# fabian-sp/GGLasso

Measured on AMD Instinct MI355X. Metric: ADMM iters/sec on (K=32,p=500) GGL at 1/2/4/8 GPUs; eigh HBM GB/s vs peak, higher is better.
Workload: dtype f64

## Files before the change

### gglasso_amd/csrc/capi_ops.hip

```cpp
#include "capi_internal.hpp"

static int eig_common(int K, int p, const double* A, const double* beta, double* D, double* Q, double* out, int map,
                      int eig_method)
{
    ARGCHK(K >= 1 && p >= 1 && A, "K, p, A");
    ARGCHK(eig_method != GGL_EIG_JACOBI || jacobi_fits(p), "GGL_EIG_JACOBI needs p <= GGL_JACOBI_MAX_P");
    const bool jac = (eig_method == GGL_EIG_JACOBI) || (eig_method == GGL_EIG_AUTO && jacobi_fits(p));
    const size_t n = (size_t)K * p * p, kp = (size_t)K * p;
    DevBuf dA, dD, dR, dO, dB, dE, dS;
    int* dinfo = nullptr;
    HIPCHK(dA.alloc(n));
    HIPCHK(dD.alloc(kp));
    HIPCHK(dB.alloc(K));
    HIPCHK(hipMalloc(&dinfo, K * sizeof(int)));
    struct InfoFree { int* p; ~InfoFree() { (void)hipFree(p); } } infofree{dinfo};
    UP(dA.p, A, n);
    if (beta) UP(dB.p, beta, K);
    if (out) HIPCHK(dO.alloc(n));
    std::vector<int> info(K);
    if (jac) {
        if (Q) HIPCHK(dR.alloc(n));
        HIPCHK(launch_jacobi(nullptr, dA.p, dD.p, dR.p, dO.p, map, beta ? dB.p : nullptr, dinfo, K, p));
        HIPCHK(hipDeviceSynchronize());
        HIPCHK(hipMemcpy(info.data(), dinfo, K * sizeof(int), hipMemcpyDeviceToHost));
// ... 120 lines not shown
    std::vector<double> h(n), coef((size_t)K * NS_NCOEF, 0.0);
    unsigned long long s = 88172645463325252ull;
    for (size_t i = 0; i < n; ++i) {
        s ^= s << 13; s ^= s >> 7; s ^= s << 17;
        h[i] = (double)(s >> 11) / 9007199254740992.0 - 0.5;
    }
    for (int k = 0; k < K; ++k) coef[(size_t)k * NS_NCOEF + 1] = 1.0 / p;
    DevBuf dA, dB, dC, dcoef;
    HIPCHK(dA.alloc(n));
    HIPCHK(dB.alloc(n));
    HIPCHK(dC.alloc(n));
    HIPCHK(dcoef.alloc(coef.size()));
    UP(dA.p, h.data(), n);
    UP(dB.p, h.data(), n);
    UP(dcoef.p, coef.data(), coef.size());
    hipEvent_t e0, e1;
    HIPCHK(hipEventCreate(&e0));
    HIPCHK(hipEventCreate(&e1));
    for (int i = 0; i < 3; ++i) launch_symm(nullptr, dA.p, dB.p, dC.p, nullptr, nullptr, dcoef.p, K, p, variant);
    HIPCHK(hipEventRecord(e0, nullptr));
    for (int i = 0; i < iters; ++i) launch_symm(nullptr, dA.p, dB.p, dC.p, nullptr, nullptr, dcoef.p, K, p, variant);
    HIPCHK(hipEventRecord(e1, nullptr));
    HIPCHK(hipEventSynchronize(e1));
    float ms = 0.f;
    HIPCHK(hipEventElapsedTime(&ms, e0, e1));
    (void)hipEventDestroy(e0);
    (void)hipEventDestroy(e1);
    HIPCHK(hipGetLastError());
    *ms_out = ms / iters;
    return GGL_OK;
}

#ifdef GGL_DEV
extern "C" int ggl_dev_set_symm_epilogue(int serial) { return symm_set_serial_epilogue(serial != 0) ? 1 : 0; }

extern "C" int ggl_dev_symm_bench_ops(int K, int p, int variant, int iters, int ops, double* ms_out)
{
    ARGCHK(K >= 1 && p >= 1 && iters >= 1 && ms_out && ops >= 0 && ops <= 7, "arguments");
    ARGCHK(variant < 0 || symm_variant_built(variant), "product-kernel variant not in this build");
    const size_t n = (size_t)K * p * p;
    std::vector<double> h(n), coef((size_t)K * NS_NCOEF, 0.0);
    unsigned long long s = 88172645463325252ull;
    for (size_t i = 0; i < n; ++i) {
        s ^= s << 13; s ^= s >> 7; s ^= s << 17;
        h[i] = (double)(s >> 11) / 9007199254740992.0 - 0.5;
    }
    for (int k = 0; k < K; ++k)
        for (int i = 0; i < p; ++i)
            for (int j = 0; j < i; ++j) h[((size_t)k * p + i) * p + j] = h[((size_t)k * p + j) * p + i];
    for (int k = 0; k < K; ++k) {
        double* c = coef.data() + (size_t)k * NS_NCOEF;
        c[0] = 1.5; c[1] = 1.0 / p; c[2] = -0.5; c[3] = 0.25; c[4] = 0.5; c[5] = 0.125; c[6] = 0.75; c[7] = -0.375;
    }
    DevBuf dA, dB, dC, dC2, dcoef;
    HIPCHK(dA.alloc(n));
    HIPCHK(dB.alloc(n));
    HIPCHK(dC.alloc(n));
    HIPCHK(dC2.alloc(n));
    HIPCHK(dcoef.alloc(coef.size()));
    UP(dA.p, h.data(), n);
    UP(dB.p, h.data(), n);
    UP(dcoef.p, coef.data(), coef.size());
    const double* E = (ops & 1) ? dA.p : nullptr;
    const double* E2 = (ops & 2) ? dB.p : nullptr;
    double* C2 = (ops & 4) ? dC2.p : nullptr;
    struct Events {
        hipEvent_t e0 = nullptr, e1 = nullptr;
// ... 907 lines not shown
```

### gglasso_amd/csrc/gemm_sym.hip

```cpp
#include <algorithm>
#include <initializer_list>
#include <mutex>
#include <unordered_map>
#include <type_traits>

#include "common.hpp"
#include "kernels.hpp"
#include "sym_tile.hpp"

namespace ggl {


__device__ __forceinline__ double c2val(double dC, double v, double dE, double e) { return __builtin_fma(dE, e, dC * v); }
__device__ __forceinline__ double c2val2(double dC, double v, double dE, double e, bool has2, double dE2, double f)
{
    const double w = c2val(dC, v, dE, e);
    return has2 ? __builtin_fma(dE2, f, w) : w;
}


template <int BM, int BK, int WM, int WN, bool LM, int ABL = 0>
__global__ __launch_bounds__(sym_nt(BM, WM, WN)) void k_symm_tn(
    const double* __restrict__ A, const double* __restrict__ B, double* __restrict__ C, double* __restrict__ C2,
    const double* __restrict__ E, const double* __restrict__ coef, int K, int p, const double* __restrict__ A1,
    const double* __restrict__ B1, double* __restrict__ C1, int K1, double* __restrict__ maxdev,
    const double* __restrict__ E2)
{
    using Cfg = SymCfg<BM, BK, WM, WN, LM>;
    __shared__ __attribute__((aligned(16))) double smem[Cfg::LDS_DOUBLES];
    double* As = smem;
    double* Bs = smem + Cfg::SLAB;
    const int T = (p + BM - 1) / BM;
    int k, b;
    if (!decode_block_xcd(T * (T + 1) / 2, K + K1, k, b)) return;
    const bool second = k >= K;
    const int kk = second ? k - K : k;
    int I = 0;
    while (b >= T - I) { b -= T - I; ++I; }
    const int J = I + b;
    const int I0 = I * BM, J0 = J * BM;
    const int tid = threadIdx.x, lane = tid & 63, wave = tid >> 6;
    const int wr = (wave / Cfg::NWC) * WM, wc = (wave % Cfg::NWC) * WN;
    const size_t pp = (size_t)p * p;
    const double* Ak = (second ? A1 : A) + (size_t)kk * pp;
    const double* Bk = (second ? B1 : B) + (size_t)kk * pp;

#ifdef GGL_DEV
    long long t_start = 0, t_loop = 0, t_loop_end = 0;
    if (ABL == 3) t_start = clock64();
#endif

    v4d acc[Cfg::TI][Cfg::TJ];
// ... 304 lines not shown
            for (int j = 0; j < IPW; ++j) {
                const int i = wave * IPW + j;
                const unsigned ro = min((unsigned)(m0 + RPI * i + lrow), pm1) * pu;
                double* la = base + j * 128;
                __builtin_amdgcn_global_load_lds((gptr_t)(Ak + ro + ca), (lptr_t)la, 16, 0, AUX);
                __builtin_amdgcn_global_load_lds((gptr_t)(Bk + ro + cb), (lptr_t)(la + SLAB), 16, 0, AUX);
            }
        }
    };
    constexpr bool REBAL = (TI == 2 && TJ == 2 && NW == 4);
    int rbk[TI], cbk[TJ];
#pragma unroll
    for (int i = 0; i < TI; ++i) rbk[i] = wr + 16 * i;
#pragma unroll
    for (int j = 0; j < TJ; ++j) cbk[j] = wc + 16 * j;
    const bool skipU = REBAL && I == J;
    int nval = TI * TJ;
    if (skipU) {
        nval = 3;
        if (wave == 1) { cbk[0] = wc + 16; cbk[TJ - 1] = wc; }
        else if (wave == 2) { rbk[0] = 16; rbk[TI - 1] = 0; cbk[0] = WN + 16; cbk[TJ - 1] = WN; nval = 1; }
    }
    const bool dead_wave = !REBAL && (I == J) && (wr >= wc + WN);
    double cI = 0.0, cAcc = 0.0, cE = 0.0, dI = 0.0, dC = 0.0, dE = 0.0, cE2 = 0.0, dE2 = 0.0;
    double* Ck = (second ? C1 : C) + (size_t)kk * pp;
    double* C2k = (C2 && !second) ? C2 + (size_t)kk * pp : nullptr;
    const double* Ek = (E && !second) ? E + (size_t)kk * pp : nullptr;
    const double* E2k = (E2 && !second) ? E2 + (size_t)kk * pp : nullptr;
    auto load_coefs = [&] {
        cI = coef[k * NS_NCOEF + 0]; cAcc = coef[k * NS_NCOEF + 1]; cE = coef[k * NS_NCOEF + 2];
        dI = coef[k * NS_NCOEF + 3]; dC = coef[k * NS_NCOEF + 4]; dE = coef[k * NS_NCOEF + 5];
        cE2 = E2k ? coef[k * NS_NCOEF + 6] : 0.0; dE2 = E2k ? coef[k * NS_NCOEF + 7] : 0.0;
    };
    if constexpr (SER == 0 && ABL != 4) load_coefs();
    const int S = (p + BK - 1) / BK;
#pragma unroll
    for (int q = 0; q < NSTG - 1; ++q)
        if (q < S) issue(q, q);
    const int fg = lane >> 4, fsw = 16 * (fg & 1);
    const double* pfa[TI];
    const double* pfb[TJ];
#pragma unroll
    for (int i = 0; i < TI; ++i) pfa[i] = smem + fg * BM + ((rbk[i] + (lane & 15)) ^ fsw);
#pragma unroll
    for (int j = 0; j < TJ; ++j) pfb[j] = smem + SLAB + fg * BM + ((cbk[j] + (lane & 15)) ^ fsw);
    auto slab = [&](const int s, auto bufc) {
        constexpr int buf = decltype(bufc)::value;
        const int ahead = min(NSTG - 2, S - 1 - s);
        if (NSTG >= 6 && ahead >= 4) wait_vmcnt<(NSTG >= 6 ? 8 * IPW : 0)>();
        else if (NSTG >= 5 && ahead >= 3) wait_vmcnt<(NSTG >= 5 ? 6 * IPW : 0)>();
        else if (NSTG >= 4 && ahead >= 2) wait_vmcnt<4 * IPW>();
        else if (NSTG >= 3 && ahead >= 1) wait_vmcnt<2 * IPW>();
        else wait_vmcnt<0>();
        const int valid = p - s * BK;
        if (valid < BK) {
            for (int e = lane; e < RPW * BM; e += 64) {
                const int row = wave * RPW + e / BM;
                if (row >= valid) {
                    smem[(size_t)buf * 2 * SLAB + row * BM + (e % BM)] = 0.0;
                    smem[(size_t)buf * 2 * SLAB + SLAB + row * BM + (e % BM)] = 0.0;
                }
            }
        }
        asm volatile("s_waitcnt lgkmcnt(0)" ::: "memory");
        if (ABL != 5) __builtin_amdgcn_s_barrier();
        asm volatile("" ::: "memory");
        if (s + NSTG - 1 < S) issue(s + NSTG - 1, (buf + NSTG - 1) % NSTG);
// ... 11 lines not shown
                for (int i = 0; i < TI; ++i) af[i] = pfa[i][so + kq4 * 4 * BM];
#pragma unroll
                for (int j = 0; j < TJ; ++j) bf[j] = pfb[j][so + kq4 * 4 * BM];
                if constexpr (REBAL && ABL != 3) {
                    if (!skipU) acc[TI - 1][0] = __builtin_amdgcn_mfma_f64_16x16x4f64(af[TI - 1], bf[0], acc[TI - 1][0], 0, 0, 0);
                    acc[0][0] = __builtin_amdgcn_mfma_f64_16x16x4f64(af[0], bf[0], acc[0][0], 0, 0, 0);
                    acc[0][TJ - 1] = __builtin_amdgcn_mfma_f64_16x16x4f64(af[0], bf[TJ - 1], acc[0][TJ - 1], 0, 0, 0);
                    acc[TI - 1][TJ - 1] = __builtin_amdgcn_mfma_f64_16x16x4f64(af[TI - 1], bf[TJ - 1], acc[TI - 1][TJ - 1], 0, 0, 0);
                } else {
#pragma unroll
                    for (int i = 0; i < TI; ++i)
#pragma unroll
                        for (int j = 0; j < TJ; ++j) {
                            if (ABL == 3) { acc[i][j][0] += af[i] * bf[j]; continue; }
                            acc[i][j] = __builtin_amdgcn_mfma_f64_16x16x4f64(af[i], bf[j], acc[i][j], 0, 0, 0);
                        }
                }
            }
#if defined(GGL_EXP_SETPRIO) && GGL_EXP_SETPRIO == 1
            __builtin_amdgcn_s_setprio(0);
#endif
        }
    };
    auto stages = [&](const int s0, auto... bufs) {
        (void)std::initializer_list<int>{((s0 + (int)decltype(bufs)::value < S) ? (slab(s0 + (int)decltype(bufs)::value, bufs), 0) : 0)...};
    };
    static_assert(NSTG == 2 || NSTG == 3 || NSTG == 4 || NSTG == 6, "stage counts with an unrolled slab loop");
    for (int s0 = 0; s0 < S; s0 += NSTG) {
        if constexpr (NSTG == 2) stages(s0, std::integral_constant<int, 0>{}, std::integral_constant<int, 1>{});
        else if constexpr (NSTG == 3) stages(s0, std::integral_constant<int, 0>{}, std::integral_constant<int, 1>{}, std::integral_constant<int, 2>{});
        else if constexpr (NSTG == 4) stages(s0, std::integral_constant<int, 0>{}, std::integral_constant<int, 1>{}, std::integral_constant<int, 2>{}, std::integral_constant<int, 3>{});
        else stages(s0, std::integral_constant<int, 0>{}, std::integral_constant<int, 1>{}, std::integral_constant<int, 2>{}, std::integral_constant<int, 3>{}, std::integral_constant<int, 4>{}, std::integral_constant<int, 5>{});
    }
    if constexpr (ABL == 4 || SER != 0) __syncthreads();
#if defined(GGL_EXP_SETPRIO) && GGL_EXP_SETPRIO == 2
    __builtin_amdgcn_s_setprio(2);
#endif
    if (ABL == 4) {
        double keepalive = 0.0;
#pragma unroll
        for (int i = 0; i < TI; ++i)
#pragma unroll
            for (int j = 0; j < TJ; ++j) keepalive += acc[i][j][0] + acc[i][j][1] + acc[i][j][2] + acc[i][j][3];
        if (keepalive == 1234.5678) C[0] = keepalive;
        return;
    }

#ifdef GGL_DEV
    if constexpr (SER != 0) {
        load_coefs();
        double dev = 0.0;
        const bool wide = (I != J) && ABL != 1;
        if (wide) {
    #pragma unroll
            for (int ti = 0; ti < TI; ++ti)
    #pragma unroll
                for (int tj = 0; tj < TJ; ++tj)
    #pragma unroll
                    for (int r = 0; r < 4; ++r) {
                        const int row = wr + ti * 16 + (lane >> 4) + 4 * r;
                        const int col = wc + tj * 16 + (lane & 15);
                        smem[row * BM + (col ^ row)] = cAcc * acc[ti][tj][r];
                    }
            __syncthreads();
            auto ld2 = [](const double* q) { return *reinterpret_cast<const double2*>(q); };
            auto lde2 = [&](const double* q) {
                if constexpr (AUX == 0) return *reinterpret_cast<const double2*>(q);
                else { double2 e; e.x = ld_pol<AUX>(q); e.y = ld_pol<AUX>(q + 1); return e; }
            };
            for (int e2 = tid; e2 < BM * BM / 2; e2 += NT) {
                const int row = e2 / (BM / 2), c2 = (e2 % (BM / 2)) * 2;
                const int gi = I0 + row, gj = J0 + c2;
                double2 t = ld2(smem + row * BM + ((c2 ^ row) & ~1));
                if (row & 1) { const double h = t.x; t.x = t.y; t.y = h; }
                if (gi < p && gj + 1 < p) {
                    double2 e = {0.0, 0.0}, f = {0.0, 0.0};
                    if (Ek) e = lde2(Ek + (size_t)gi * p + gj);
                    if (E2k) f = lde2(E2k + (size_t)gi * p + gj);
                    double2 v;
                    v.x = t.x + cE * e.x;
                    v.y = t.y + cE * e.y;
                    if (E2k) { v.x += cE2 * f.x; v.y += cE2 * f.y; }
// ... 108 lines not shown
                    const double f0 = need_f ? ld_pol<AUX>(E2k + (size_t)(J0 + a) * p + I0 + c2) : 0.0;
                    if (!rowpart) { v0 += cE * e0; if (E2k) v0 += cE2 * f0; }
                    Ck[(size_t)(J0 + a) * p + I0 + c2] = v0;
                    if (C2k) C2k[(size_t)(J0 + a) * p + I0 + c2] = c2val2(dC, v0, dE, e0, E2k != nullptr, dE2, f0);
                }
            }
        }
        return;
    }
#endif
    constexpr int LDSB = NSTG * 2 * SLAB * 8;
    constexpr int WGCU = (160 * 1024 / LDSB) < (8 / (NW / 4)) ? (160 * 1024 / LDSB) : (8 / (NW / 4));
    constexpr int VBUD = (512 / (WGCU * (NW / 4))) & ~7;
    constexpr int BREG = VBUD - TI * TJ * 8 - 48 - XREG;
    constexpr int NTRIP = BM * BM / 2 / NT;
    constexpr int NB = (BREG / 8 >= NTRIP) ? NTRIP : (BREG / 8 >= NTRIP / 2 && NTRIP >= 2) ? NTRIP / 2 : 1;
    constexpr int NBLK = TI * TJ;
    constexpr int DB = (BREG / 16 >= NBLK) ? NBLK : (BREG / 16 >= NBLK / 2 && NBLK >= 2) ? NBLK / 2 : 1;
    static_assert(NTRIP * NT * 2 == BM * BM && NTRIP % NB == 0 && NBLK % DB == 0, "epilogue batches");
    auto lds_barrier = [] {
        asm volatile("s_waitcnt lgkmcnt(0)" ::: "memory");
        __builtin_amdgcn_s_barrier();
        asm volatile("" ::: "memory");
    };
    auto landed = [](const double& x) { asm volatile("" ::"v"(x)); };
    auto landed2 = [&](const double2& x) { landed(x.x); landed(x.y); };
    auto ld2 = [](const double* q) { return *reinterpret_cast<const double2*>(q); };
    auto lde2 = [&](const double* q) {
        if constexpr (AUX == 0) return *reinterpret_cast<const double2*>(q);
        else { double2 e; e.x = ld_pol<AUX>(q); e.y = ld_pol<AUX>(q + 1); return e; }
    };
    double dev = 0.0;
    const bool wide = (I != J) && ABL != 1;
    if (wide) {
        double2 pe[NB], pf[NB];
        auto direct_loads = [&](const int u0) {
#pragma unroll
            for (int q = 0; q < NB; ++q) {
                const int e2 = tid + (u0 + q) * NT;
                const int row = e2 / (BM / 2), c2 = (e2 % (BM / 2)) * 2;
                const int gi = I0 + row, gj = J0 + c2;
                const bool any = gi < p && gj < p, half = any && gj + 1 >= p;
                const size_t o = (size_t)gi * p + gj - (half ? 1 : 0);
                pe[q] = double2{0.0, 0.0};
                pf[q] = double2{0.0, 0.0};
                if (any) {
                    if (Ek) pe[q] = lde2(Ek + o);
                    if (E2k) pf[q] = lde2(E2k + o);
                }
            }
        };
        direct_loads(0);
        lds_barrier();
#pragma unroll
        for (int ti = 0; ti < TI; ++ti)
#pragma unroll
            for (int tj = 0; tj < TJ; ++tj)
#pragma unroll
                for (int r = 0; r < 4; ++r) {
                    const int row = wr + ti * 16 + (lane >> 4) + 4 * r;
                    const int col = wc + tj * 16 + (lane & 15);
                    smem[row * BM + (col ^ row)] = cAcc * acc[ti][tj][r];
                }
        lds_barrier();
#pragma unroll
        for (int u0 = 0; u0 < NTRIP; u0 += NB) {
            if (u0 > 0) direct_loads(u0);
// ... 82 lines not shown
            for (int q = 0; q < DB; ++q) {
                const int ti = (b0 + q) / TJ, tj = (b0 + q) % TJ;
                if (no_block(ti, tj)) continue;
#pragma unroll
                for (int r = 0; r < 4; ++r) {
                    const int row = rbk[ti] + (lane >> 4) + 4 * r;
                    const int col = cbk[tj] + (lane & 15);
                    const int gi = I0 + row, gj = J0 + col;
                    double v = cAcc * acc[ti][tj][r];
                    const bool keep = gi < p && gj < p && (I != J || gi <= gj);
                    if (keep) {
                        if (gi == gj) v += cI;
                        const double e0 = de[q * 4 + r], f0 = df[q * 4 + r];
                        v = __builtin_fma(cE, e0, v);
                        if (E2k) v = __builtin_fma(cE2, f0, v);
                        dev = fmax(dev, fabs(v - (gi == gj ? 1.0 : 0.0)));
                        Ck[(size_t)gi * p + gj] = v;
                        if (C2k) C2k[(size_t)gi * p + gj] = c2val2(dC, v, dE, e0, E2k != nullptr, dE2, f0) + (gi == gj ? dI : 0.0);
                        if (I == J && gi != gj) {
                            Ck[(size_t)gj * p + gi] = v;
                            if (C2k) C2k[(size_t)gj * p + gi] = c2val2(dC, v, dE, e0, E2k != nullptr, dE2, f0);
                        }
                    }
                    if ((I != J || rowpart) && ABL != 1) smem[row * BM + (col ^ row)] = (rowpart && !keep) ? 0.0 : v;
                }
            }
        }
    }
    if (maxdev) {
        dev = wave_max(dev);
        if (lane == 0 && dev > 0.0)
            atomicMax(reinterpret_cast<unsigned long long*>(maxdev + k), (unsigned long long)__double_as_longlong(dev));
    }
    if ((I != J || rowpart) && ABL != 1) lds_barrier();
    if (rowpart && ABL != 1 && tid < 2 * BM) symm_dl_partials<BM>(smem, rowpart, fropart, k, p, T, blockTile, I, J, I0, J0, tid);
    if (wide) {
        const bool need_e = Ek && C2k && (!rowpart || dE != 0.0), need_f = E2k && C2k && (!rowpart || dE2 != 0.0);
        double2 me[NB], mf[NB];
#pragma unroll
        for (int u0 = 0; u0 < NTRIP; u0 += NB) {
#pragma unroll
            for (int q = 0; q < NB; ++q) {
                const int e2 = tid + (u0 + q) * NT;
                const int a = e2 / (BM / 2), c2 = (e2 % (BM / 2)) * 2;
                const size_t o = (size_t)(J0 + a) * p + I0 + c2;
                const bool any = J0 + a < p && I0 + c2 < p, half = any && I0 + c2 + 1 >= p;
                me[q] = double2{0.0, 0.0};
                mf[q] = double2{0.0, 0.0};
                if (any) {
                    if (need_e) me[q] = lde2(Ek + o - (half ? 1 : 0));
                    if (need_f) mf[q] = lde2(E2k + o - (half ? 1 : 0));
                }
            }
#pragma unroll
            for (int q = 0; q < NB; ++q) { landed2(me[q]); landed2(mf[q]); }
#pragma unroll
            for (int q = 0; q < NB; ++q) {
                const int e2 = tid + (u0 + q) * NT;
                const int a = e2 / (BM / 2), c2 = (e2 % (BM / 2)) * 2;
                const size_t o = (size_t)(J0 + a) * p + I0 + c2;
                double2 e = me[q], f = mf[q];
                if (J0 + a < p && I0 + c2 < p && I0 + c2 + 1 >= p) { e.x = e.y; f.x = f.y; }
                if (J0 + a < p && I0 + c2 + 1 < p) {
                    double2 v;
                    v.x = smem[c2 * BM + (a ^ c2)];
                    v.y = smem[(c2 + 1) * BM + (a ^ (c2 + 1))];
                    *reinterpret_cast<double2*>(Ck + o) = v;
                    if (C2k) {
                        double2 w;
// ... 461 lines not shown
                    if (Ek && dE != 0.0) e = *reinterpret_cast<const double2*>(Ek + (size_t)gm * p + gc);
                    double2 w2;
                    w2.x = c2val(dC, v.x, dE, e.x);
                    w2.y = c2val(dC, v.y, dE, e.y);
                    *reinterpret_cast<double2*>(C2k + (size_t)gm * p + gc) = w2;
                }
            }
        }
    }
    if (rowpart && tid < 2 * BM) {
        const int t = tid & (BM - 1);
        const bool second = tid >= BM;
        double rs = 0.0, sq = 0.0;
        if (!second) {
#pragma unroll 8
            for (int c = 0; c < BM; ++c) { const double x = smem[t * BM + ((c + t) & (BM - 1))]; rs += fabs(x); sq += x * x; }
        } else if (I != J) {
#pragma unroll 8
            for (int r = 0; r < BM; ++r) rs += fabs(smem[((r + t) & (BM - 1)) * BM + t]);
        }
        if (I != J) sq *= 2.0;
        if (I != J || !second) {
            const int slot = second ? I : J, gr = (second ? J0 : I0) + t;
            if (gr < p) rowpart[((size_t)k * T + slot) * (size_t)p + gr] = rs;
        }
        sq = wave_sum(second ? 0.0 : sq);
        if (tid == 0) fropart[(size_t)k * (T * (T + 1) / 2) + blockTile] = sq;
    }
}

#endif

#ifdef GGL_DEV
static bool g_symm_serial = false;
bool symm_set_serial_epilogue(bool on) { const bool was = g_symm_serial; g_symm_serial = on; return was; }
#endif

#ifdef GGL_DEV
template <int BK, int NSTG, int BM, int AUX, int SER = 0>
__global__ __launch_bounds__(256) void k_omega_chain(const ChainProg P, unsigned* __restrict__ state)
{
    __shared__ __attribute__((aligned(16))) double smem[NSTG * 2 * BK * BM];
    __shared__ int sh_job[3];
    __shared__ unsigned char sh_step[CHAIN_MAX_INST];
    unsigned xcc;
    asm volatile("s_getreg_b32 %0, hwreg(HW_REG_XCC_ID)" : "=s"(xcc));
    const int x = (int)(xcc & 0xfu) % NXCD;
    const int ninst = min((P.K - x + NXCD - 1) / NXCD, CHAIN_MAX_INST);
    const int rot = ninst > 0 ? (int)(blockIdx.x / NXCD) % ninst : 0;
    unsigned backoff = 4;
    if (threadIdx.x < CHAIN_MAX_INST) sh_step[threadIdx.x] = 0;
#ifdef GGL_DEV
    long long t_claim = 0, t_idle = 0, t_tile = 0, n_tile = 0, t_prev = wall_clock64(), t_first = t_prev;
    const long long c_first = clock64();
#endif
    __syncthreads();
    for (;;) {
        if (threadIdx.x == 0) {
            int jk = -2, js = 0, jb = 0;
            for (int ii = 0; ii < ninst && jk < 0; ++ii) {
                const int i = (ii + rot) % ninst;
                const int k = x + NXCD * i;
                unsigned* w = state + (size_t)k * CHAIN_CNT_STRIDE;
                int s = sh_step[i];
                while (s < P.nops) {
                    const unsigned nt = (unsigned)(P.begin[s + 1] - P.begin[s]);
                    const unsigned t = __hip_atomic_fetch_add(w + 1 + s, 1u, __ATOMIC_RELAXED, __HIP_MEMORY_SCOPE_WORKGROUP);
                    if (t < nt) { jk = k; js = s; jb = (int)t; break; }
// ... 2 lines not shown
                    ++s;
                }
                sh_step[i] = (unsigned char)s;
            }
            sh_job[0] = jk; sh_job[1] = js; sh_job[2] = jb;
        }
        __syncthreads();
        const int jk = __builtin_amdgcn_readfirstlane(sh_job[0]);
        const int js = __builtin_amdgcn_readfirstlane(sh_job[1]);
        int jb = __builtin_amdgcn_readfirstlane(sh_job[2]);
        __syncthreads();
#ifdef GGL_DEV
        if (jk == -2 && P.prof && threadIdx.x == 0) {
            long long* o = P.prof + (size_t)blockIdx.x * 8;
            o[0] = t_claim; o[1] = t_idle; o[2] = t_tile; o[3] = n_tile; o[4] = t_first; o[5] = wall_clock64(); o[6] = x; o[7] = clock64() - c_first;
        }
#endif
        if (jk == -2) return;
        if (jk == -1) {
            for (unsigned q = 0; q < backoff; ++q) __builtin_amdgcn_s_sleep(8);
            backoff = min(backoff * 2u, 64u);
#ifdef GGL_DEV
            { const long long t = wall_clock64(); t_idle += t - t_prev; t_prev = t; }
#endif
            continue;
        }
        backoff = 4;
#ifdef GGL_DEV
        { const long long t = wall_clock64(); t_claim += t - t_prev; t_prev = t; }
#endif
        const SymmOp& o = P.op[js];
        int kk = jk;
        if (o.pair && jb >= P.ntiles) { kk = P.K + jk; jb -= P.ntiles; }
        symm_dl_tile<BK, NSTG, 0, BM, 4, AUX, SER, 32>(o.A, o.B, o.C, o.C2, o.E, o.E2, o.coef, P.K, P.p, o.A1, o.B1, o.C1, o.pair ? P.K : 0,
                                               nullptr, o.rowpart, o.fropart, kk, jb, smem);
        asm volatile("s_waitcnt vmcnt(0)" ::: "memory");
        __syncthreads();
        if (threadIdx.x == 0)
            __hip_atomic_fetch_add(state + (size_t)jk * CHAIN_CNT_STRIDE, 1u, __ATOMIC_RELAXED, __HIP_MEMORY_SCOPE_WORKGROUP);
#ifdef GGL_DEV
        { const long long t = wall_clock64(); t_tile += t - t_prev; t_prev = t; n_tile += 1; }
#endif
    }
}

__global__ __launch_bounds__(64) void k_chain_check(const unsigned* __restrict__ state, int K, unsigned total,
                                                    int* __restrict__ flag, int* __restrict__ flag_h)
{
    bool bad = false;
    for (int k = threadIdx.x; k < K; k += 64) bad = bad || (state[(size_t)k * CHAIN_CNT_STRIDE] != total);
    if (__any(bad) && threadIdx.x == 0) { *flag = 1; *flag_h = 1; }
}

int chain_tile(int K, int p, bool force)
{
    if ((p & 1) != 0 || K < NXCD || K > NXCD * CHAIN_MAX_INST) return 0;
    const long T = (p + 63) / 64;
    return (force || T * (T + 1) / 2 * K >= 1100) ? 64 : 0;
}

int launch_omega_chain(hipStream_t st, const ChainProg& P, unsigned* state, int* flag, int* flag_h, int aux)
{
    static int slots = 0;
    if (!slots) {
        int dev = 0, per_cu = 0;
        hipDeviceProp_t prop;
        if (hipGetDevice(&dev) != hipSuccess || hipGetDeviceProperties(&prop, dev) != hipSuccess) return -1;
        if (hipOccupancyMaxActiveBlocksPerMultiprocessor(&per_cu, (const void*)k_omega_chain<16, 3, 64, 16>, 256, 0) != hipSuccess || per_cu < 1)
            return -1;
        slots = std::min(per_cu, 3) * prop.multiProcessorCount;
        slots -= slots % NXCD;
    }
    if (aux == 0) hipLaunchKernelGGL((k_omega_chain<16, 3, 64, 0>), dim3(slots), dim3(256), 0, st, P, state);
    else if (g_symm_serial) hipLaunchKernelGGL((k_omega_chain<16, 3, 64, 16, 1>), dim3(slots), dim3(256), 0, st, P, state);
    else
    hipLaunchKernelGGL((k_omega_chain<16, 3, 64, 16>), dim3(slots), dim3(256), 0, st, P, state);
    hipLaunchKernelGGL(k_chain_check, dim3(1), dim3(64), 0, st, state, P.K, (unsigned)P.begin[P.nops], flag, flag_h);
    return slots;
}

__device__ __forceinline__ void grid_barrier(unsigned* counter, unsigned target, unsigned* err)
{
    __syncthreads();
    if (threadIdx.x == 0) {
        __builtin_amdgcn_fence(__ATOMIC_RELEASE, "agent");
        __hip_atomic_fetch_add(counter, 1u, __ATOMIC_RELAXED, __HIP_MEMORY_SCOPE_AGENT);
        long spins = 0;
        while (__hip_atomic_load(counter, __ATOMIC_RELAXED, __HIP_MEMORY_SCOPE_AGENT) < target) {
            __builtin_amdgcn_s_sleep(1);
            if (++spins > (1L << 22)) {
                __hip_atomic_store(err, 1u, __ATOMIC_RELAXED, __HIP_MEMORY_SCOPE_AGENT);
                break;
            }
        }
        __builtin_amdgcn_fence(__ATOMIC_ACQUIRE, "agent");
    }
    __syncthreads();
}

__device__ __forceinline__ void grid_barrier_xcd(unsigned* bar, unsigned phase, unsigned per_xcd, unsigned xcd)
{
    __syncthreads();
    if (threadIdx.x == 0) {
        const unsigned old = __hip_atomic_fetch_add(bar + 8 + xcd, 1u, __ATOMIC_RELAXED, __HIP_MEMORY_SCOPE_AGENT);
        if (old + 1 == phase * per_xcd) {
            __builtin_amdgcn_fence(__ATOMIC_RELEASE, "agent");
            __hip_atomic_fetch_add(bar, 1u, __ATOMIC_RELAXED, __HIP_MEMORY_SCOPE_AGENT);
// ... 79 lines not shown
    if (g_red_rider.nblk > 0) {
        launch_reduce_partials(st, g_red_rider.partials, 1, g_red_rider.nblk, g_red_rider.nv, g_red_rider.out, g_red_rider.seq,
                               g_red_rider.seq_val);
        g_red_rider = RedRider{};
    }
    if (g_copy_rider.n > 0) {
        launch_copy_small(st, g_copy_rider);
        g_copy_rider = CopySegs{};
    }
    if (g_rider.K <= 0) return;
    hipLaunchKernelGGL(k_cw_rider, dim3(g_rider.K * g_rider.nbx), dim3(256), 0, st, g_rider);
    g_rider = CwRider{};
}

static void launch_dl(hipStream_t st, const double* A, const double* B, double* C, double* C2, const double* E,
                      const double* coef, int K, int p, const double* A1, const double* B1, double* C1, int K1,
                      double* maxdev, int dl_cfg = 0, double* rowpart = nullptr, double* fropart = nullptr,
                      const double* E2 = nullptr)
{
    const bool eight = dl_cfg == 6 || dl_cfg == 7;
    const CwRider rider = (g_rider.K > 0 && !eight) ? g_rider : CwRider{};
    if (rider.K > 0) g_rider = CwRider{};
    const CopySegs cps = (g_copy_rider.n > 0 && !eight) ? g_copy_rider : CopySegs{};
    if (cps.n > 0) g_copy_rider = CopySegs{};
    const RedRider red = (g_red_rider.nblk > 0 && !eight) ? g_red_rider : RedRider{};
    if (red.nblk > 0) g_red_rider = RedRider{};
    int ncopy = red.nblk > 0 ? NXCD : 0;
    for (int i = 0; i < cps.n; ++i) ncopy += (int)((cps.words[i] + 1023u) / 1024u);
    const int nride = rider.K * rider.nbx + ncopy;
#define GGL_DL_ARGS A, B, C, C2, E, E2, coef, K, p, A1, B1, C1, K1, maxdev, rowpart, fropart, rider, cps, red
#ifdef GGL_DEV
#define GGL_DL4(BK_, NSTG_, ABL_, BM_)                                                                                        \
    do {                                                                                                                       \
        if (g_symm_serial) hipLaunchKernelGGL((k_symm_dl<BK_, NSTG_, ABL_, BM_, 4, 1>), grid, dim3(256), 0, st, GGL_DL_ARGS); \
        else hipLaunchKernelGGL((k_symm_dl<BK_, NSTG_, ABL_, BM_, 4, 0>), grid, dim3(256), 0, st, GGL_DL_ARGS);               \
    } while (0)
#else
#define GGL_DL4(BK_, NSTG_, ABL_, BM_) hipLaunchKernelGGL((k_symm_dl<BK_, NSTG_, ABL_, BM_>), grid, dim3(256), 0, st, GGL_DL_ARGS)
#endif
#define GGL_DL3(BK_, NSTG_, ABL_) GGL_DL4(BK_, NSTG_, ABL_, 64)
#define GGL_DL2(BK_, NSTG_) GGL_DL4(BK_, NSTG_, 0, 64)
#define GGL_DL_PICK(a1, a2, a3, a4, NAME, ...) NAME
#define GGL_DL(...) GGL_DL_PICK(__VA_ARGS__, GGL_DL4, GGL_DL3, GGL_DL2, )(__VA_ARGS__)
    if (dl_cfg == 4 || (dl_cfg >= 8 && dl_cfg <= 13) || (dl_cfg >= 18 && dl_cfg <= 21)) {
        const int T32 = (p + 31) / 32;
        const dim3 grid(xcd_grid(T32 * (T32 + 1) / 2, K + K1) + nride);
        if (dl_cfg == 4) GGL_DL(32, 2, 0, 32);
#ifdef GGL_DEV
        else if (dl_cfg == 8) GGL_DL(16, 4, 0, 32);
        else if (dl_cfg == 9) GGL_DL(32, 3, 0, 32);
        else if (dl_cfg == 10) GGL_DL(16, 6, 0, 32);
        else if (dl_cfg == 11) GGL_DL(32, 4, 0, 32);
        else if (dl_cfg == 12) GGL_DL(16, 2, 0, 32);
        else if (dl_cfg == 13) GGL_DL(16, 3, 0, 32);
        else if (dl_cfg == 18) GGL_DL(32, 2, 2, 32);
        else if (dl_cfg == 19) GGL_DL(32, 2, 3, 32);
        else if (dl_cfg == 20) GGL_DL(32, 2, 4, 32);
        else if (dl_cfg == 21) GGL_DL(32, 2, 5, 32);
#endif
        return;
    }
    const int T = (p + 63) / 64;
    const dim3 grid(xcd_grid(T * (T + 1) / 2, K + K1) + nride);
#ifdef GGL_DEV
    if (dl_cfg == 6 || dl_cfg == 7) {
#define GGL_DL8(BK_, NSTG_)                                                                                                   \
    do {                                                                                                                       \
        if (g_symm_serial) hipLaunchKernelGGL((k_symm_dl<BK_, NSTG_, 0, 64, 8, 1>), grid, dim3(512), 0, st, GGL_DL_ARGS);     \
        else hipLaunchKernelGGL((k_symm_dl<BK_, NSTG_, 0, 64, 8, 0>), grid, dim3(512), 0, st, GGL_DL_ARGS);                   \
    } while (0)
        if (dl_cfg == 6) GGL_DL8(16, 4);
        else GGL_DL8(32, 3);
#undef GGL_DL8
        return;
    }
#endif
    if (dl_cfg == 1) GGL_DL(16, 3);
#ifdef GGL_DEV
    else if (dl_cfg == 2) GGL_DL(16, 4);
    else if (dl_cfg == 3) GGL_DL(32, 2);
    else if (dl_cfg == 5) GGL_DL(16, 2, 1);
    else if (dl_cfg == 14) GGL_DL(16, 3, 2);
    else if (dl_cfg == 15) GGL_DL(16, 3, 3);
    else if (dl_cfg == 16) GGL_DL(16, 3, 4);
    else if (dl_cfg == 17) GGL_DL(16, 3, 5);
    else if (dl_cfg == 22) GGL_DL(8, 4);
    else if (dl_cfg == 23) GGL_DL(8, 6);
#endif
    else GGL_DL(16, 2);
#undef GGL_DL
#undef GGL_DL_PICK
#undef GGL_DL2
#undef GGL_DL3
#undef GGL_DL4
#undef GGL_DL_ARGS
}

template <int BM, int BK, int WM, int WN>
__global__ __launch_bounds__(sym_nt(BM, WM, WN)) void k_gemm_nt_right(const double* __restrict__ A,
                                                                      const double* __restrict__ T,
                                                                      double* __restrict__ C,
// ... 386 lines not shown
```

### gglasso_amd/csrc/kernels.hpp

```cpp
#pragma once
#include <hip/hip_runtime.h>
#include <stddef.h>

#define GGL_NNORM 5

namespace ggl {

enum EigMap {
    MAP_PHIPLUS = 0,
    MAP_RANK = 1,
    MAP_IDENT = 2
};

int elementwise_blocks(int p);
void launch_form_W(hipStream_t st, double* W, const double* Theta, const double* L, const double* X,
                   const double* S, const double* betaK, int K, int p);
void launch_theta_sgl(hipStream_t st, double* Theta, double* X, double* C, const double* Omega,
                      const double* OmegaPrev, const double* L, const double* l1K,
                      const double* mask, const double* invrhoK, int latent, double* partials, int K, int p, const int* skip = nullptr,
                      const int* pk = nullptr, size_t mask_stride = 0);
void launch_dual_update(hipStream_t st, double* X, const double* Omega, const double* OmegaPrev,
                        const double* Theta, const double* L, double* partials, int K, int p);
void launch_reduce_partials(hipStream_t st, const double* partials, int K, int nblk, int nv, double* out,
                            unsigned long long* seq = nullptr, unsigned long long seq_val = 0, unsigned* arrive = nullptr);
// ... 144 lines not shown
    double *wscale = nullptr, *wscale_h = nullptr;
    int* flag = nullptr;
};
struct I8Cfg { int s_full = 7, s_f2 = 4, s_gf2 = 3, s_ye = 5, d_ye = 4; };
struct I8Bufs { const double* W; double *Ap, *Bp, *Y1, *F, *F2, *Om; };
struct I8Prog {
    struct Prod { I8Op op; int SA, SB, dmax; } prod[I8_MAXPROD];
    int nprod = 0, units = 0, k0 = 0, Kp = 0, S_W = 7;
};
int i8_omega_alloc(I8Omega* w, int K, int p);
void i8_omega_free(I8Omega* w);
int i8_omega_plan(I8Omega* w, const double* cuse_h, const double* beta_h, int k0, int Kp, double tol, int degrees,
                  const I8Cfg& cfg, const I8Bufs& bufs, I8Prog* prog);
bool i8_omega_run(hipStream_t st, I8Omega* w, const I8Prog& prog, const double* W);
hipError_t launch_jacobi(hipStream_t st, const double* A, double* D, double* R, double* out, int map,
                         const double* betaK, int* info, int K, int p);

void launch_recon(hipStream_t st, double* out, const double* R, const double* D, const double* betaK,
                  int map, int K, int p, double* scale_work);

static constexpr int NS_NCOEF = 8;
int symm_variants();
bool symm_variant_built(int v);
bool symm_dl_serves(int p);
void symm_set_odd_dl(bool on);
int symm_effective_variant(int variant, int p);
int symm_auto_variant(int nprod, int p);
void launch_symm(hipStream_t st, const double* A, const double* B, double* C, double* C2, const double* E,
                 const double* coef, int K, int p, int variant, double* maxdev = nullptr, double* rowpart = nullptr,
                 double* fropart = nullptr, const double* E2 = nullptr);
int symm_bounds_tile(int K, int p, int variant);
void symm_release_workspace(hipStream_t st);
#ifdef GGL_DEV
bool symm_set_serial_epilogue(bool on);
#endif

struct SymmOp {
    const double *A, *B, *E, *A1, *B1, *E2;
    double *C, *C2, *C1;
    const double* coef;
    double *rowpart, *fropart;
    int pair, pad_;
};
static constexpr int CHAIN_MAX_OPS = 16;
struct ChainProg {
    int nops, K, p, ntiles;
    int begin[CHAIN_MAX_OPS + 1];
    SymmOp op[CHAIN_MAX_OPS];
    long long* prof = nullptr;
};
int chain_tile(int K, int p, bool force = false);
static constexpr int CHAIN_CNT_STRIDE = 32;
static constexpr int CHAIN_MAX_INST = 64;
static_assert(CHAIN_MAX_OPS + 1 <= CHAIN_CNT_STRIDE, "one line holds the completion word and the ticket words");
int launch_omega_chain(hipStream_t st, const ChainProg& P, unsigned* state, int* flag, int* flag_h, int aux = 16);

#ifdef GGL_DEV
int launch_chain_probe(hipStream_t st, double* X0, double* X1, const double* coef, int K, int p, int nprod, int variant,
                       unsigned* bar, unsigned* err, int two_level);
#endif
#ifdef GGL_DEV
void coissue_probe(hipStream_t st, double* scratch, double* out);
void mfma_lds_probe(hipStream_t st, double* scratch, double* out);
#endif
double mfma_f64_peak_tflops(hipStream_t st, double* scratch, int blocks, int iters, int nacc);
double mfma_valu_mix_tflops(hipStream_t st, double* scratch, int blocks, int iters, int nv);
void launch_gemm_right(hipStream_t st, const double* A, const double* T, double* C, const double* scal,
// ... 147 lines not shown
```

### include/ggl_hip.h

```cpp
#ifndef GGL_HIP_H
#define GGL_HIP_H

#ifdef __cplusplus
extern "C" {
#endif

#define GGL_VERSION 300

#define GGL_OK 0
#define GGL_E_ARG (-1)
#define GGL_E_HIP (-2)
#define GGL_E_SOLVER (-3)
#define GGL_E_ALLOC (-4)
#define GGL_E_COMM (-5)

#define GGL_REG_SGL 0
#define GGL_REG_GGL 1
#define GGL_REG_FGL 2
#define GGL_REG_FSGL 3

#define GGL_EIG_AUTO 0
#define GGL_EIG_JACOBI 1
#define GGL_EIG_ROCSOLVER 2
#define GGL_EIG_NEWTON_SCHULZ 3
// ... 189 lines not shown
int ggl_fsgl_stats(ggl_ctx *ctx, long long out[4]);
int ggl_trace_start(ggl_ctx *ctx, int max_events);
int ggl_trace_read(ggl_ctx *ctx, double *out, int cap);
int ggl_eig_info(ggl_ctx *ctx, int *out);

int ggl_dev_symm(int K, int p, const double *A, const double *B, const double *E, const double *coef5K,
                 double *C, double *C2, int variant);
int ggl_dev_symm_bench(int K, int p, int variant, int iters, double *ms_out);
int ggl_dev_omega_lds(int K, int p, const double *Theta, const double *L, const double *X, const double *S, const double *beta,
                      double tol, int degrees, double *Omega, double *cbound, int iters, double *out);
int ggl_dev_symm_bounds(int K, int p, const double *A, const double *B, int variant, double *C,
                        double *rowsum_out, double *fro2_out, double *bound_out);
int ggl_dev_ns_schedule(double l, int degrees, int max_steps, int *deg_out, double *coef_out, int *units_out);
int ggl_dev_ns_schedule_tol(double l, int degrees, double tol, int max_steps, int *deg_out, double *coef_out,
                            int *units_out);
int ggl_dev_group_partition(const int *units, int K, int p, int max_groups, int *len_out);
int ggl_dev_ns_units(double l, int degrees, double tol);
int ggl_dev_omega_poly_plan(double a, double tol, int degrees, int *deg, double *out, int *units);
#ifdef GGL_DEV
int ggl_dev_i8_stages(int n);
int ggl_dev_symm_i8(int K, int p, int S, int dmax, const double *A, const double *B, double scaleA, double scaleB, double *C,
                    int iters, double *ms_out);
int ggl_dev_omega_i8(int K, int p, const double *W, const double *beta, const double *cbound, const int *cfg5, double tol,
                     double *Omega, int iters, double *ms_out);
int ggl_dev_mfma_f64_peak(double *tflops_out);
int ggl_dev_coissue_probe(double *out12);
int ggl_dev_mfma_lds_probe(double *out6);
int ggl_dev_chain_run(int K, int p, int nprod, int iters, double *out);
int ggl_dev_switch_bench(int K, int p, int variant, int iters, int mode, double *ms_out);
int ggl_dev_vendor_bench(int K, int p, int mode, int iters, double *ms_out);
int ggl_dev_fill_copy_probe(int reps, int K, int p, int slices, int gap_us, long long out[2]);
int ggl_dev_symm_timeline(int K, int p, long long *out, int max_blocks, int *nblocks_out);
int ggl_dev_chain_probe(int K, int p, int variant, int nprod, int iters, int two_level, double *out);
int ggl_dev_set_symm_epilogue(int serial);
int ggl_dev_symm_bench_ops(int K, int p, int variant, int iters, int ops, double *ms_out);
int ggl_dev_symm_full(int K, int p, const double *A, const double *B, const double *E, const double *E2, const double *coef8K,
                      double *C, double *C2, int variant);
#endif

int ggl_eigh_batched(int K, int p, const double *A, double *D, double *Q, int eig_method);
int ggl_phiplus(int K, int p, const double *beta, const double *D, const double *Q, double *out);
int ggl_prox_rank_norm(int K, int p, const double *beta, const double *D, const double *Q, double *out);
int ggl_phiplus_matrix(int K, int p, const double *beta, const double *W, double *out, int eig_method);
int ggl_rank_matrix(int K, int p, const double *beta, const double *C, double *out, int eig_method);
int ggl_rank_matrix_ex(int K, int p, const double *beta, const double *C, double *out, int eig_method, double l0_coarse,
                       long long stats[6]);
int ggl_rank_matrix_deflate(int K, int p, const double *beta, const double *C, double *out, int eig_method, double l0_deflate,
                            long long stats[8]);
int ggl_prox_od_1norm(int p, const double *A, double lam, const double *lam_pp, double *out);
int ggl_prox_sum_frob(int p, int M, const double *X, double l, double *out);
int ggl_frob_norm_per_block(int p, int M, const double *S, int off_diag, double *out);
int ggl_prox_p(int K, int p, const double *X, double l1, double l2, int reg, double *out);
int ggl_prox_tv(int n, int K, const double *Y, double lam, double *out);
int ggl_prox_2norm(int n, int K, const double *Y, double lam, double *out);
int ggl_prox_phi(int n, int K, const double *Y, double l1, double l2, int reg, double *out);

#define GGL_COV_CENTER 1
#define GGL_COV_SCALE 2
#define GGL_COV_TILE32 4
#define GGL_COV_TILE64 8
int ggl_covariance(int device, int K, int p, const int *N, const double *const *X_host, int flags, double *S_out,
                   double *scale_out);
int ggl_scale_by_diagonal(int device, int K, int p, const double *X_host, const double *d_in, double *Y_out, double *d_out);
int ggl_set_S_from_data(ggl_ctx *ctx, const double *const *X_host, const int *N, int flags);
int ggl_get_S(ggl_ctx *ctx, double *S_out, double *scale_out);

int ggl_covariance_subsets(int device, int p, int N, const double *X_host, int B, int b, const int *idx, int flags,
// ... 45 lines not shown
```

Baseline: 1539.

## Add register-resident symmetric-product epilogue using DPP and permlane16 swaps

For off-diagonal tiles of the symmetric product kernel, a new epilogue applies the coefficient combination and writes both the tile and its mirrored transpose straight from registers. It uses lane_xor1 (DPP) and permlane16_swap cross-lane shuffles instead of staging accumulators through LDS. This skips the LDS barrier and the LDS round-trip for those tiles, and the E/E2 loads are issued in register batches. The old LDS epilogue is kept as dev mode 2, and the chain kernel is pinned to it. The risks are higher register pressure and less coalesced mirrored stores.

```diff
diff --git a/gglasso_amd/csrc/capi_ops.hip b/gglasso_amd/csrc/capi_ops.hip
--- a/gglasso_amd/csrc/capi_ops.hip
+++ b/gglasso_amd/csrc/capi_ops.hip
@@ -176,7 +176,7 @@
 }
 
 #ifdef GGL_DEV
-extern "C" int ggl_dev_set_symm_epilogue(int serial) { return symm_set_serial_epilogue(serial != 0) ? 1 : 0; }
+extern "C" int ggl_dev_set_symm_epilogue(int mode) { return symm_set_epilogue(mode); }
 
 extern "C" int ggl_dev_symm_bench_ops(int K, int p, int variant, int iters, int ops, double* ms_out)
 {
diff --git a/gglasso_amd/csrc/gemm_sym.hip b/gglasso_amd/csrc/gemm_sym.hip
--- a/gglasso_amd/csrc/gemm_sym.hip
+++ b/gglasso_amd/csrc/gemm_sym.hip
@@ -18,6 +18,21 @@
     return has2 ? __builtin_fma(dE2, f, w) : w;
 }
 
+__device__ __forceinline__ double lane_xor1(double x)
+{
+    const unsigned long long b = (unsigned long long)__double_as_longlong(x);
+    const unsigned lo = (unsigned)__builtin_amdgcn_update_dpp(0, (int)(unsigned)b, 0xB1, 0xf, 0xf, true);
+    const unsigned hi = (unsigned)__builtin_amdgcn_update_dpp(0, (int)(unsigned)(b >> 32), 0xB1, 0xf, 0xf, true);
+    return __longlong_as_double((long long)(((unsigned long long)hi << 32) | lo));
+}
+__device__ __forceinline__ void swap_row16(double& a, double& b)
+{
+    const unsigned long long x = (unsigned long long)__double_as_longlong(a), y = (unsigned long long)__double_as_longlong(b);
+    const auto lo = __builtin_amdgcn_permlane16_swap((unsigned)x, (unsigned)y, false, false);
+    const auto hi = __builtin_amdgcn_permlane16_swap((unsigned)(x >> 32), (unsigned)(y >> 32), false, false);
+    a = __longlong_as_double((long long)(((unsigned long long)hi[0] << 32) | lo[0]));
+    b = __longlong_as_double((long long)(((unsigned long long)hi[1] << 32) | lo[1]));
+}
 
 template <int BM, int BK, int WM, int WN, bool LM, int ABL = 0>
 __global__ __launch_bounds__(sym_nt(BM, WM, WN)) void k_symm_tn(
@@ -388,7 +403,7 @@
         dI = coef[k * NS_NCOEF + 3]; dC = coef[k * NS_NCOEF + 4]; dE = coef[k * NS_NCOEF + 5];
         cE2 = E2k ? coef[k * NS_NCOEF + 6] : 0.0; dE2 = E2k ? coef[k * NS_NCOEF + 7] : 0.0;
     };
-    if constexpr (SER == 0 && ABL != 4) load_coefs();
+    if constexpr (SER != 1 && ABL != 4) load_coefs();
     const int S = (p + BK - 1) / BK;
 #pragma unroll
     for (int q = 0; q < NSTG - 1; ++q)
@@ -466,7 +481,7 @@
         else if constexpr (NSTG == 4) stages(s0, std::integral_constant<int, 0>{}, std::integral_constant<int, 1>{}, std::integral_constant<int, 2>{}, std::integral_constant<int, 3>{});
         else stages(s0, std::integral_constant<int, 0>{}, std::integral_constant<int, 1>{}, std::integral_constant<int, 2>{}, std::integral_constant<int, 3>{}, std::integral_constant<int, 4>{}, std::integral_constant<int, 5>{});
     }
-    if constexpr (ABL == 4 || SER != 0) __syncthreads();
+    if constexpr (ABL == 4 || SER == 1) __syncthreads();
 #if defined(GGL_EXP_SETPRIO) && GGL_EXP_SETPRIO == 2
     __builtin_amdgcn_s_setprio(2);
 #endif
@@ -481,7 +496,7 @@
     }
 
 #ifdef GGL_DEV
-    if constexpr (SER != 0) {
+    if constexpr (SER == 1) {
         load_coefs();
         double dev = 0.0;
         const bool wide = (I != J) && ABL != 1;
@@ -656,7 +671,95 @@
     };
     double dev = 0.0;
     const bool wide = (I != J) && ABL != 1;
-    if (wide) {
+    constexpr bool REGEP = (SER == 0) && NB >= 2;
+    const bool regs = REGEP && wide && !rowpart;
+    if (regs) {
+        constexpr int RB = DB;
+        const int g = lane >> 4, odd = lane & 1, cc = lane & 14;
+        const size_t o00 = (size_t)(I0 + wr + g + 8 * odd) * p + (size_t)(J0 + wc + cc);
+        const size_t m00 = (size_t)(J0 + wc + cc) * p + (size_t)(I0 + wr + 2 * (g >> 1) + 4 * (g & 1) + 8 * odd);
+        double2 re[RB * 2], rf[RB * 2];
+        auto reg_loads = [&](const int b0) {
+#pragma unroll
+            for (int q = 0; q < RB; ++q) {
+                const int ti = (b0 + q) / TJ, tj = (b0 + q) % TJ;
+                const int gj = J0 + wc + 16 * tj + cc;
+                const bool any = gj < p, half = any && gj + 1 >= p;
+#pragma unroll
+                for (int h = 0; h < 2; ++h) {
+                    const size_t o = o00 + (size_t)(16 * ti + 4 * h) * p + 16 * tj - (half ? 1 : 0);
+                    re[q * 2 + h] = double2{0.0, 0.0};
+                    rf[q * 2 + h] = double2{0.0, 0.0};
+                    if (any) {
+                        if (Ek) re[q * 2 + h] = lde2(Ek + o);
+                        if (E2k) rf[q * 2 + h] = lde2(E2k + o);
+                    }
+                }
+            }
+        };
+        auto exchange = [&](const int blk, double2* t) {
+            const int ti = blk / TJ, tj = blk % TJ;
+#pragma unroll
+            for (int h = 0; h < 2; ++h) {
+                const double lo = cAcc * acc[ti][tj][h], hi = cAcc * acc[ti][tj][2 + h];
+                const double plo = lane_xor1(lo), phi = lane_xor1(hi);
+                t[h].x = odd ? phi : lo;
+                t[h].y = odd ? hi : plo;
+            }
+        };
+        reg_loads(0);
+#pragma unroll
+        for (int b0 = 0; b0 < NBLK; b0 += RB) {
+            if (b0 > 0) reg_loads(b0);
+            double2 t0[2];
+            exchange(b0, t0);
+#pragma unroll
+            for (int q = 0; q < RB * 2; ++q) { landed2(re[q]); landed2(rf[q]); }
+#pragma unroll
+            for (int q = 0; q < RB; ++q) {
+                const int ti = (b0 + q) / TJ, tj = (b0 + q) % TJ;
+                const int gj = J0 + wc + 16 * tj + cc;
+                const bool any = gj < p, full = gj + 1 < p;
+                double2 t[2], v[2], w[2];
+                if (q == 0) { t[0] = t0[0]; t[1] = t0[1]; }
+                else exchange(b0 + q, t);
+#pragma unroll
+                for (int h = 0; h < 2; ++h) {
+                    const size_t o = o00 + (size_t)(16 * ti + 4 * h) * p + 16 * tj;
+                    double2 e = re[q * 2 + h], f = rf[q * 2 + h];
+                    if (any && !full) { e.x = e.y; f.x = f.y; }
+                    v[h].x = __builtin_fma(cE, e.x, t[h].x);
+                    v[h].y = __builtin_fma(cE, e.y, t[h].y);
+                    if (E2k) { v[h].x = __builtin_fma(cE2, f.x, v[h].x); v[h].y = __builtin_fma(cE2, f.y, v[h].y); }
+                    w[h] = double2{0.0, 0.0};
+                    if (C2k) {
+                        w[h].x = c2val(dC, v[h].x, dE, e.x);
+                        w[h].y = c2val(dC, v[h].y, dE, e.y);
+                        if (E2k) { w[h].x = __builtin_fma(dE2, f.x, w[h].x); w[h].y = __builtin_fma(dE2, f.y, w[h].y); }
+                    }
+                    dev = fmax(dev, fmax(any ? fabs(v[h].x) : 0.0, full ? fabs(v[h].y) : 0.0));
+                    if (full) {
+                        *reinterpret_cast<double2*>(Ck + o) = v[h];
+                        if (C2k) *reinterpret_cast<double2*>(C2k + o) = w[h];
+                    } else if (any) {
+                        Ck[o] = v[h].x;
+                        if (C2k) C2k[o] = w[h].x;
+                    }
+                }
+                const size_t mo = m00 + (size_t)(16 * tj) * p + 16 * ti;
+                swap_row16(v[0].x, v[1].x);
+                swap_row16(v[0].y, v[1].y);
+                if (any) *reinterpret_cast<double2*>(Ck + mo) = double2{v[0].x, v[1].x};
+                if (full) *reinterpret_cast<double2*>(Ck + mo + p) = double2{v[0].y, v[1].y};
+                if (C2k) {
+                    swap_row16(w[0].x, w[1].x);
+                    swap_row16(w[0].y, w[1].y);
+                    if (any) *reinterpret_cast<double2*>(C2k + mo) = double2{w[0].x, w[1].x};
+                    if (full) *reinterpret_cast<double2*>(C2k + mo + p) = double2{w[0].y, w[1].y};
+                }
+            }
+        }
+    } else if (wide) {
         double2 pe[NB], pf[NB];
         auto direct_loads = [&](const int u0) {
 #pragma unroll
@@ -805,9 +908,9 @@
         if (lane == 0 && dev > 0.0)
             atomicMax(reinterpret_cast<unsigned long long*>(maxdev + k), (unsigned long long)__double_as_longlong(dev));
     }
-    if ((I != J || rowpart) && ABL != 1) lds_barrier();
+    if ((I != J || rowpart) && ABL != 1 && !regs) lds_barrier();
     if (rowpart && ABL != 1 && tid < 2 * BM) symm_dl_partials<BM>(smem, rowpart, fropart, k, p, T, blockTile, I, J, I0, J0, tid);
-    if (wide) {
+    if (wide && !regs) {
         const bool need_e = Ek && C2k && (!rowpart || dE != 0.0), need_f = E2k && C2k && (!rowpart || dE2 != 0.0);
         double2 me[NB], mf[NB];
 #pragma unroll
@@ -1335,8 +1438,13 @@
 #endif
 
 #ifdef GGL_DEV
-static bool g_symm_serial = false;
-bool symm_set_serial_epilogue(bool on) { const bool was = g_symm_serial; g_symm_serial = on; return was; }
+static int g_symm_epilogue = 0;
+int symm_set_epilogue(int mode)
+{
+    const int was = g_symm_epilogue;
+    g_symm_epilogue = (mode == 1 || mode == 2) ? mode : 0;
+    return was;
+}
 #endif
 
 #ifdef GGL_DEV
@@ -1405,7 +1513,7 @@
         const SymmOp& o = P.op[js];
         int kk = jk;
         if (o.pair && jb >= P.ntiles) { kk = P.K + jk; jb -= P.ntiles; }
-        symm_dl_tile<BK, NSTG, 0, BM, 4, AUX, SER, 32>(o.A, o.B, o.C, o.C2, o.E, o.E2, o.coef, P.K, P.p, o.A1, o.B1, o.C1, o.pair ? P.K : 0,
+        symm_dl_tile<BK, NSTG, 0, BM, 4, AUX, SER == 0 ? 2 : SER, 32>(o.A, o.B, o.C, o.C2, o.E, o.E2, o.coef, P.K, P.p, o.A1, o.B1, o.C1, o.pair ? P.K : 0,
                                                nullptr, o.rowpart, o.fropart, kk, jb, smem);
         asm volatile("s_waitcnt vmcnt(0)" ::: "memory");
         __syncthreads();
@@ -1445,7 +1553,7 @@
         slots -= slots % NXCD;
     }
     if (aux == 0) hipLaunchKernelGGL((k_omega_chain<16, 3, 64, 0>), dim3(slots), dim3(256), 0, st, P, state);
-    else if (g_symm_serial) hipLaunchKernelGGL((k_omega_chain<16, 3, 64, 16, 1>), dim3(slots), dim3(256), 0, st, P, state);
+    else if (g_symm_epilogue == 1) hipLaunchKernelGGL((k_omega_chain<16, 3, 64, 16, 1>), dim3(slots), dim3(256), 0, st, P, state);
     else
     hipLaunchKernelGGL((k_omega_chain<16, 3, 64, 16>), dim3(slots), dim3(256), 0, st, P, state);
     hipLaunchKernelGGL(k_chain_check, dim3(1), dim3(64), 0, st, state, P.K, (unsigned)P.begin[P.nops], flag, flag_h);
@@ -1591,7 +1699,8 @@
 #ifdef GGL_DEV
 #define GGL_DL4(BK_, NSTG_, ABL_, BM_)                                                                                        \
     do {                                                                                                                       \
-        if (g_symm_serial) hipLaunchKernelGGL((k_symm_dl<BK_, NSTG_, ABL_, BM_, 4, 1>), grid, dim3(256), 0, st, GGL_DL_ARGS); \
+        if (g_symm_epilogue == 1) hipLaunchKernelGGL((k_symm_dl<BK_, NSTG_, ABL_, BM_, 4, 1>), grid, dim3(256), 0, st, GGL_DL_ARGS); \
+        else if (g_symm_epilogue == 2) hipLaunchKernelGGL((k_symm_dl<BK_, NSTG_, ABL_, BM_, 4, 2>), grid, dim3(256), 0, st, GGL_DL_ARGS); \
         else hipLaunchKernelGGL((k_symm_dl<BK_, NSTG_, ABL_, BM_, 4, 0>), grid, dim3(256), 0, st, GGL_DL_ARGS);               \
     } while (0)
 #else
@@ -1625,7 +1734,8 @@
     if (dl_cfg == 6 || dl_cfg == 7) {
 #define GGL_DL8(BK_, NSTG_)                                                                                                   \
     do {                                                                                                                       \
-        if (g_symm_serial) hipLaunchKernelGGL((k_symm_dl<BK_, NSTG_, 0, 64, 8, 1>), grid, dim3(512), 0, st, GGL_DL_ARGS);     \
+        if (g_symm_epilogue == 1) hipLaunchKernelGGL((k_symm_dl<BK_, NSTG_, 0, 64, 8, 1>), grid, dim3(512), 0, st, GGL_DL_ARGS); \
+        else if (g_symm_epilogue == 2) hipLaunchKernelGGL((k_symm_dl<BK_, NSTG_, 0, 64, 8, 2>), grid, dim3(512), 0, st, GGL_DL_ARGS); \
         else hipLaunchKernelGGL((k_symm_dl<BK_, NSTG_, 0, 64, 8, 0>), grid, dim3(512), 0, st, GGL_DL_ARGS);                   \
     } while (0)
         if (dl_cfg == 6) GGL_DL8(16, 4);
diff --git a/gglasso_amd/csrc/kernels.hpp b/gglasso_amd/csrc/kernels.hpp
--- a/gglasso_amd/csrc/kernels.hpp
+++ b/gglasso_amd/csrc/kernels.hpp
@@ -200,7 +200,7 @@
 int symm_bounds_tile(int K, int p, int variant);
 void symm_release_workspace(hipStream_t st);
 #ifdef GGL_DEV
-bool symm_set_serial_epilogue(bool on);
+int symm_set_epilogue(int mode);
 #endif
 
 struct SymmOp {
diff --git a/include/ggl_hip.h b/include/ggl_hip.h
--- a/include/ggl_hip.h
+++ b/include/ggl_hip.h
@@ -245,7 +245,7 @@
 int ggl_dev_fill_copy_probe(int reps, int K, int p, int slices, int gap_us, long long out[2]);
 int ggl_dev_symm_timeline(int K, int p, long long *out, int max_blocks, int *nblocks_out);
 int ggl_dev_chain_probe(int K, int p, int variant, int nprod, int iters, int two_level, double *out);
-int ggl_dev_set_symm_epilogue(int serial);
+int ggl_dev_set_symm_epilogue(int mode);
 int ggl_dev_symm_bench_ops(int K, int p, int variant, int iters, int ops, double *ms_out);
 int ggl_dev_symm_full(int K, int p, const double *A, const double *B, const double *E, const double *E2, const double *coef8K,
                       double *C, double *C2, int variant);
```

Result: faster. 1568 (median of 6 runs) (+1.9%).
